# tjiangHIT/cuteSV

Measured on NVIDIA H100. Metric: sv_signatures_clustered_per_sec, higher is better.
Workload: dtype int32

## Files before the change

cutesv_b200/csrc/cutesv_b200.cu:

```cuda
#include <cuda_runtime.h>
#include <dlfcn.h>
#include <nccl.h>
#include <stdarg.h>
#include <stdio.h>
#include <stdlib.h>
#include <string.h>

#include <algorithm>
#include <atomic>
#include <string>
#include <vector>

#include "../../include/cutesv_b200.h"
#include "core.h"
#include "devprims.cuh"
#include "host_tables.h"
#include "kernels.cuh"
#include "radix.cuh"
#include "extract.cuh"
#include "scan_core.h"
#include "sa_core.h"

using namespace csv;

// ... 1050 lines not shown
    if (gs != s) {
        CU(cudaEventRecord(c->ev_side_join[side_k], gs));
        CU(cudaStreamWaitEvent(s, c->ev_side_join[side_k], 0));
    }
    stage_end(c, s, CSV_ST_CLUSTER);
    if (L.mark >= 0) { CU(cudaEventRecord(c->kivs[L.mark].b, s)); L.mark = -1; }
    return CSV_OK;
}

static int run_indel(csv_ctx* c, Lane& L, int t, uint32_t kslot_base) {
    SigTable& s = c->sig[t];
    const cudaStream_t st = L.stream;
    const int64_t n = s.n;
    const uint64_t total = c->contig_off[c->n_contigs];
    const int bits = bits_for(total);
    const bool k64 = bits > 32;
    ContigTab ct{c->d_off.as<uint64_t>(), c->d_len_eff.as<int64_t>(), c->n_contigs};
    Counters* ctr = c->counters.as<Counters>();
    TypeJob J;
    memset(&J, 0, sizeof(J));
    J.svtype = t; J.n_host = n; J.n_dev = nullptr;
    J.cp = cluster_params(c->P, t);
    const uint32_t radius = (uint32_t)std::min<int64_t>((int64_t)(J.cp.min_support - 1) * J.cp.bias, 1 << 24);
    const double lambda = (double)n * (2.0 * radius + 2.0 * (1 << BKT_SHIFT)) / (double)std::max<uint64_t>(total, 1);
    const int rb = (int)((radius + (1u << BKT_SHIFT) - 1) >> BKT_SHIFT);
    const bool prefilter = !k64 && c->prefilter_enabled && J.cp.min_support >= 3 && lambda < 0.8 * J.cp.min_support &&
                           n >= (1 << 16) && rb <= BKT_PAD;
    J.iv.rec = nullptr; J.iv.recc = nullptr;
    uint32_t* sidx = nullptr;
    int rc;
    if (prefilter) {
        int W = PART_W_MAX;
        while (W > PART_W_MIN && (int64_t)(total >> W) + 1 < 2 * (int64_t)c->n_sm) W--;
        const int P = (int)(total >> W) + 1;
        const int n_chunks = (int)((n + PART_ROUND - 1) / PART_ROUND);
        const uint32_t ptw = (uint32_t)((n + PART_PAGE - 1) / PART_PAGE) + 1;
        const size_t edge_words = (size_t)PART_MAX * 2 * BKT_PAD, tab_words = PART_MAX + (size_t)P * ptw;
        stage_begin(c, st, CSV_ST_KEYS);
        CU(L.boff.ensure((edge_words + tab_words) * 4, true));
        uint32_t* edge = L.boff.as<uint32_t>();
        uint32_t* fill = edge + edge_words;
        uint32_t* pt = fill + PART_MAX;
        CU(L.keys_a.ensure(((size_t)ptw - 1 + P) * PART_PAGE * 8));
        uint2* pool = (uint2*)L.keys_a.p;
        CU(L.rec_a.ensure((size_t)n * sizeof(IndelRec)));
        CU(cudaMemsetAsync(edge, 0, (size_t)P * 2 * BKT_PAD * 4, st));
        const int is_ins = t == CSV_INS ? 1 : 0;
        if ((((uintptr_t)s.chrom.p) | ((uintptr_t)s.a.p)) & 15)
            return set_err(CSV_E_STATE, "signature columns are not 16 B aligned");
        uint32_t* pool_next = nullptr;
        TileSync ts;
        if ((rc = take_ticket(c->lb, &pool_next)) || (rc = make_sync(c->lb, L.lb_status, st, (size_t)P, &ts))) return rc;
        const size_t smem = pf_smem_bytes(W);
        const int g = std::min(P, resident_grid(c, k_part_filter, 256, smem));
        LAUNCH(c, st, k_part_scatter, n_chunks, PS_THREADS, ps_smem_bytes(), s.chrom.as<int32_t>(), s.a.as<int32_t>(), n, is_ins, ct, W, P,
               rb, pool, fill, pt, ptw, pool_next, edge, &ctr->status);
        stage_end(c, st, CSV_ST_KEYS);
        stage_begin(c, st, CSV_ST_SORT);
        uint32_t* n_pass = &ctr->n_dom[t];
        LAUNCH_PDL(c, st, k_part_filter, g, 256, smem, (const uint2*)pool, fill, pt, ptw, P, W, rb, (uint32_t)J.cp.min_support,
                   (const uint32_t*)edge, L.keys_b.as<uint32_t>(), L.vals_b.as<uint32_t>(), (uint2*)L.rec_a.p, n_pass, ts);
        stage_end(c, st, CSV_ST_SORT);
        if (c->lane_marks) {
            kprof_begin(c, st, t == CSV_DEL ? "back end<DEL>" : "back end<INS>");
            L.mark = (int)c->kivs.size() - 1;
        }
        J.n_dev = n_pass;
        J.keys32 = L.keys_b.as<uint32_t>();
        sidx = L.vals_b.as<uint32_t>();
    } else {
        stage_begin(c, st, CSV_ST_KEYS);
        if (!k64)
            LAUNCH(c, st, (k_indel_keys<uint32_t>), grid_for(c, n, 256), 256, 0, s.chrom.as<int32_t>(), s.a.as<int32_t>(), s.b.as<int32_t>(),
                   s.rid.as<int32_t>(), n, t == CSV_INS ? 1 : 0, ct, L.keys_a.as<uint32_t>(), &ctr->status);
        else
            LAUNCH(c, st, (k_indel_keys<uint64_t>), grid_for(c, n, 256), 256, 0, s.chrom.as<int32_t>(), s.a.as<int32_t>(), s.b.as<int32_t>(),
                   s.rid.as<int32_t>(), n, t == CSV_INS ? 1 : 0, ct, L.keys_a.as<uint64_t>(), &ctr->status);
        stage_end(c, st, CSV_ST_KEYS);
        stage_begin(c, st, CSV_ST_SORT);
        if (!k64) {
            uint32_t* ko = nullptr;
            rc = lane_sort<uint32_t>(c, L, true, n, bits, &ko, &sidx);
            J.keys32 = ko;
        } else {
            uint64_t* ko = nullptr;
            rc = lane_sort<uint64_t>(c, L, true, n, bits, &ko, &sidx);
            J.keys64 = ko;
        }
        if (rc) return rc;
        stage_end(c, st, CSV_ST_SORT);
    }
    J.iv.chrom = s.chrom.as<int32_t>(); J.iv.a = s.a.as<int32_t>(); J.iv.b = s.b.as<int32_t>(); J.iv.rid = s.rid.as<int32_t>();
    J.iv.c = s.has_c ? s.c.as<int32_t>() : nullptr;
    J.iv.sidx = sidx;
    if (!k64 && c->records_enabled && (J.cp.min_support + 31) / 32 + 1 <= HEAD_MAX_NEED_WORDS) {
        const bool with_c = t == CSV_INS && s.has_c;
        CU(L.rec_a.ensure((size_t)n * sizeof(IndelRec)));
        if (with_c) CU(L.recc_a.ensure((size_t)n * 4));
        J.iv.rec = L.rec_a.as<IndelRec>();
        J.iv.recc = with_c ? L.recc_a.as<int32_t>() : nullptr;
    }
    J.iv.is_ins = t == CSV_INS ? 1 : 0;
    J.small_path = c->small_path_enabled ? 1 : 0;
    L.prev_is_chain_kernel = prefilter;
    rc = run_segment_and_cluster(c, L, J, t, kslot_base);
    L.prev_is_chain_kernel = false;
    return rc;
}

static int run_other(csv_ctx* c, Lane& L, int t, uint32_t kslot_base) {
    SigTable& s = c->sig[t];
    const cudaStream_t st = L.stream;
    const int64_t n = s.n;
// ... 537 lines not shown
```

cutesv_b200/csrc/devprims.cuh:

```cuda
#pragma once
#include <cuda_runtime.h>
#include <stdint.h>

namespace csv {

__device__ __forceinline__ void pdl_wait() { asm volatile("griddepcontrol.wait;" ::: "memory"); }
__device__ __forceinline__ void pdl_launch_dependents() { asm volatile("griddepcontrol.launch_dependents;" ::: "memory"); }

__device__ __forceinline__ uint32_t smem_u32(const void* p) { return (uint32_t)__cvta_generic_to_shared(p); }
__device__ __forceinline__ void mbar_init(uint64_t* bar, uint32_t count) {
    asm volatile("mbarrier.init.shared::cta.b64 [%0], %1;" ::"r"(smem_u32(bar)), "r"(count) : "memory");
}
__device__ __forceinline__ void mbar_arrive(uint64_t* bar) {
    asm volatile("mbarrier.arrive.shared::cta.b64 _, [%0];" ::"r"(smem_u32(bar)) : "memory");
}
__device__ __forceinline__ void mbar_expect_tx(uint64_t* bar, uint32_t bytes) {
    asm volatile("mbarrier.arrive.expect_tx.shared::cta.b64 _, [%0], %1;" ::"r"(smem_u32(bar)), "r"(bytes) : "memory");
}
__device__ __forceinline__ void bulk_copy(void* dst, const void* src, uint32_t bytes, uint64_t* bar) {
    asm volatile("cp.async.bulk.shared::cluster.global.mbarrier::complete_tx::bytes [%0], [%1], %2, [%3];" ::"r"(smem_u32(dst)), "l"(src), "r"(bytes),
                 "r"(smem_u32(bar))
                 : "memory");
}
__device__ __forceinline__ void bulk_load(void* dst, const void* src, uint32_t bytes, uint64_t* bar) {
// ... 14 lines not shown


static constexpr uint32_t LB_GEN_LIMIT = 1u << 31;
__device__ __forceinline__ uint64_t lb_word(uint32_t gen, bool inclusive, uint32_t value) {
    return ((uint64_t)gen << 33) | ((uint64_t)inclusive << 32) | value;
}
__device__ __forceinline__ bool lb_ready(uint64_t v, uint32_t gen) { return (uint32_t)(v >> 33) == gen; }
__device__ __forceinline__ bool lb_inclusive(uint64_t v) { return (v >> 32) & 1u; }
__device__ __forceinline__ uint32_t lb_value(uint64_t v) { return (uint32_t)v; }
__device__ __forceinline__ uint64_t lb_load(const uint64_t* p) {
    uint64_t v;
    asm volatile("ld.relaxed.gpu.global.u64 %0, [%1];" : "=l"(v) : "l"(p) : "memory");
    return v;
}
__device__ __forceinline__ void lb_store(uint64_t* p, uint64_t v) {
    asm volatile("st.relaxed.gpu.global.u64 [%0], %1;" ::"l"(p), "l"(v) : "memory");
}

__device__ __forceinline__ void lookback_publish(uint64_t* status, uint32_t gen, int tile, uint32_t local) {
    lb_store(status + tile, lb_word(gen, tile == 0, local));
}

__device__ __forceinline__ uint32_t lookback_wait_warp(uint64_t* status, uint32_t gen, int tile, uint32_t local) {
    const int lane = threadIdx.x & 31;
    if (tile == 0) return 0;
    uint32_t excl = 0;
    int p = tile - 1;
    while (true) {
        const int q = p - lane;
        const uint64_t v = q >= 0 ? lb_load(status + q) : lb_word(gen, true, 0u);
        const bool ready = lb_ready(v, gen);
        const uint32_t nr = __ballot_sync(0xffffffffu, !ready);
        const uint32_t inc = __ballot_sync(0xffffffffu, ready && lb_inclusive(v));
        const int first_nr = nr ? __ffs(nr) - 1 : 32;
        const int first_inc = inc ? __ffs(inc) - 1 : 32;
        const bool done = first_inc < first_nr;
        const int upto = done ? first_inc + 1 : first_nr;
        uint32_t contrib = lane < upto ? lb_value(v) : 0u;
#pragma unroll
        for (int o = 16; o > 0; o >>= 1) contrib += __shfl_xor_sync(0xffffffffu, contrib, o);
        excl += contrib;
        if (done) break;
        p -= upto;
    }
    if (lane == 0) lb_store(status + tile, lb_word(gen, true, excl + local));
    return excl;
}

__device__ __forceinline__ uint32_t lookback_exclusive_warp(uint64_t* status, uint32_t gen, int tile, uint32_t local) {
    if ((threadIdx.x & 31) == 0) lookback_publish(status, gen, tile, local);
    return lookback_wait_warp(status, gen, tile, local);
}

__device__ __forceinline__ uint32_t block_excl_scan_256(uint32_t v, uint32_t* s_warp, uint32_t* total) {
    const int lane = threadIdx.x & 31, warp = threadIdx.x >> 5;
    uint32_t incl = v;
#pragma unroll
    for (int d = 1; d < 32; d <<= 1) {
        uint32_t y = __shfl_up_sync(0xffffffffu, incl, d);
        if (lane >= d) incl += y;
    }
    if (lane == 31) s_warp[warp] = incl;
    __syncthreads();
    if (warp == 0) {
        uint32_t w = lane < 8 ? s_warp[lane] : 0;
        uint32_t wi = w;
#pragma unroll
        for (int d = 1; d < 8; d <<= 1) {
            uint32_t y = __shfl_up_sync(0xffffffffu, wi, d);
            if (lane >= d) wi += y;
        }
        if (lane < 8) s_warp[lane] = wi - w;
        if (lane == 7) s_warp[8] = wi;
    }
    __syncthreads();
    uint32_t r = s_warp[warp] + incl - v;
    *total = s_warp[8];
    __syncthreads();
    return r;
}

__device__ __forceinline__ uint32_t block_reserve_256(uint32_t cnt, uint32_t* counter, uint32_t* s_warp , int parity) {
    const int lane = threadIdx.x & 31, warp = threadIdx.x >> 5;
    uint32_t incl = cnt;
#pragma unroll
    for (int d = 1; d < 32; d <<= 1) {
        const uint32_t y = __shfl_up_sync(0xffffffffu, incl, d);
        if (lane >= d) incl += y;
    }
    uint32_t* part = s_warp + 8 * parity;
    if (lane == 31) part[warp] = incl;
    __syncthreads();
    uint32_t before = 0, total = 0;
#pragma unroll
    for (int i = 0; i < 8; i++) {
        const uint32_t t = part[i];
        before += i < warp ? t : 0u;
        total += t;
    }
    if (threadIdx.x == 0) s_warp[16] = total ? atomicAdd(counter, total) : 0u;
    __syncthreads();
    return s_warp[16] + before + incl - cnt;
}

static constexpr int SEL_THREADS = 256;
static constexpr int SEL_ITEMS = 8;
static constexpr int SEL_TILE = SEL_THREADS * SEL_ITEMS;

struct TileSync {
    uint32_t* ticket;
    uint64_t* status;
    const uint32_t* epoch;
    uint32_t ordinal;
};
static constexpr uint32_t LB_ORDINALS = 1024;
static constexpr uint32_t LB_EPOCH_LIMIT = 1u << 21;
static_assert((uint64_t)LB_EPOCH_LIMIT * LB_ORDINALS <= LB_GEN_LIMIT, "look-back generations must fit 31 bits");
__global__ void __launch_bounds__(256) k_begin(uint32_t* epoch, uint32_t* tickets, int n_tickets, uint32_t* counters, int n_counters,
                                               unsigned long long* cursor) {
    if (threadIdx.x == 0) { *epoch += 1u; *cursor = 0ull; }
    for (int i = threadIdx.x; i < n_tickets; i += 256) tickets[i] = 0u;
    for (int i = threadIdx.x; i < n_counters; i += 256) counters[i] = 0u;
}
__device__ __forceinline__ uint32_t ts_gen(const TileSync& ts) { return (*ts.epoch) * LB_ORDINALS + ts.ordinal; }

template <class Pred>
__global__ void __launch_bounds__(SEL_THREADS) k_select(Pred pred, int64_t n_host, const uint32_t* n_dev, uint32_t* out,
                                                        uint32_t out_cap, uint32_t* out_count, TileSync ts,
                                                        uint32_t* status_word, uint32_t overflow_bit) {
    __shared__ uint32_t s_warp[9];
    __shared__ uint32_t s_tile, s_excl;
    const int64_t n = n_dev ? (int64_t)*n_dev : n_host;
    const uint32_t gen = ts_gen(ts);
    while (true) {
        if (threadIdx.x == 0) s_tile = atomicAdd(ts.ticket, 1u);
        __syncthreads();
        const uint32_t tile = s_tile;
        const int64_t base = (int64_t)tile * SEL_TILE;
        if (base >= n) break;
        const int64_t i0 = base + (int64_t)threadIdx.x * SEL_ITEMS;
        uint32_t flags = 0, cnt = 0;
#pragma unroll
        for (int j = 0; j < SEL_ITEMS; j++) {
            const int64_t i = i0 + j;
            if (i < n && pred(i)) { flags |= 1u << j; cnt++; }
        }
        uint32_t total;
        const uint32_t local = block_excl_scan_256(cnt, s_warp, &total);
        if (threadIdx.x < 32) {
            const uint32_t ex = lookback_exclusive_warp(ts.status, gen, (int)tile, total);
            if (threadIdx.x == 0) {
                s_excl = ex;
                if (base + SEL_TILE >= n) *out_count = ex + total;
            }
        }
        __syncthreads();
        uint32_t o = s_excl + local;
#pragma unroll
        for (int j = 0; j < SEL_ITEMS; j++) {
            if (flags >> j & 1u) {
                if (o < out_cap) out[o] = (uint32_t)(i0 + j);
                else atomicOr(status_word, overflow_bit);
                o++;
            }
        }
        __syncthreads();
    }
}

template <int ITEMS>
__global__ void __launch_bounds__(SEL_THREADS) k_scan_excl(uint32_t* arr, int64_t n_host, const uint32_t* n_dev, const uint32_t* carry_in,
                                                           uint32_t* total_out, TileSync ts) {
    pdl_launch_dependents(); pdl_wait();
    constexpr int TILE = SEL_THREADS * ITEMS;
    __shared__ uint32_t s_warp[9];
    __shared__ uint32_t s_tile, s_excl;
    int64_t n = n_dev ? (int64_t)*n_dev : n_host;
    if (n > n_host) n = n_host;
    const uint32_t carry = carry_in ? *carry_in : 0u;
    const uint32_t gen = ts_gen(ts);
    if (n <= 0) {
        if (total_out && blockIdx.x == 0 && threadIdx.x == 0) *total_out = carry;
        return;
    }
    while (true) {
        if (threadIdx.x == 0) s_tile = atomicAdd(ts.ticket, 1u);
        __syncthreads();
        const uint32_t tile = s_tile;
        const int64_t base = (int64_t)tile * TILE;
        if (base >= n) break;
        const int64_t i0 = base + (int64_t)threadIdx.x * ITEMS;
        uint32_t v[ITEMS], cnt = 0;
        const bool vec = ITEMS == 4 && (((uintptr_t)arr) & 15) == 0 && i0 + ITEMS <= n;
        if (vec) {
            const uint4 x = *reinterpret_cast<const uint4*>(arr + i0);
            v[0] = x.x; v[1] = x.y; v[2] = x.z; v[3] = x.w;
            cnt = x.x + x.y + x.z + x.w;
        } else {
#pragma unroll
            for (int j = 0; j < ITEMS; j++) {
                v[j] = (i0 + j < n) ? arr[i0 + j] : 0u;
                cnt += v[j];
            }
        }
        uint32_t total;
        const uint32_t local = block_excl_scan_256(cnt, s_warp, &total);
        if (threadIdx.x < 32) {
            const uint32_t ex = lookback_exclusive_warp(ts.status, gen, (int)tile, total);
            if (threadIdx.x == 0) {
                s_excl = ex;
                if (total_out && base + TILE >= n) *total_out = carry + ex + total;
            }
        }
        __syncthreads();
        uint32_t run = carry + s_excl + local;
        if (vec) *reinterpret_cast<uint4*>(arr + i0) = make_uint4(run, run + v[0], run + v[0] + v[1], run + v[0] + v[1] + v[2]);
        else {
#pragma unroll
            for (int j = 0; j < ITEMS; j++) {
                if (i0 + j < n) arr[i0 + j] = run;
                run += v[j];
            }
        }
        __syncthreads();
    }
}

}
```

cutesv_b200/csrc/kernels.cuh:

```cuda
#pragma once
#include "core.h"
#include "devprims.cuh"
#include "radix.cuh"
#include <type_traits>

namespace csv {

static constexpr int WARP_M = 128;
static constexpr int BLOCK_M = 2048;
static constexpr int CL_THREADS = 256;

struct TypeJob {
    int svtype;
    int64_t n_host;
    const uint32_t* n_dev;
    const uint32_t* keys32;
    const uint64_t* keys64;
    IndelView iv;
    SortedView sv;
    ClusterParams cp;
    uint32_t kslot_base;
    const uint32_t* kept_start;
    uint32_t* big_list;
    uint32_t* giant_list;
// ... 58 lines not shown
    constexpr int WORDS = SEL_TILE / 32;
    __shared__ uint32_t s_link[HEAD_MAX_NEED_WORDS + WORDS + HEAD_MAX_NEED_WORDS];
    __shared__ uint32_t s_warp[9];
    __shared__ uint32_t s_tile, s_excl, s_aoff;
    __shared__ uint8_t s_msize[SEL_TILE];
    const int64_t n = job_n(J);
    const uint32_t gen = ts_gen(ts);
    const int need = J.cp.min_support;
    const int back = MR.rec ? (need + 31) / 32 + 1 : 0;
    const int fwd = (MR.rec ? max((need + 31) / 32, (REST_SPLIT + 32) / 32) : (need + 31) / 32) + 1;
    const int lane = threadIdx.x & 31, warp = threadIdx.x >> 5;
    while (true) {
        if (threadIdx.x == 0) s_tile = atomicAdd(ts.ticket, 1u);
        __syncthreads();
        const uint32_t tile = s_tile;
        const int64_t base = (int64_t)tile * SEL_TILE;
        if (base >= n) break;
        for (int w0 = warp; w0 < back + WORDS + fwd; w0 += 8 * (SEL_THREADS / 32)) {
            bool l[8];
#pragma unroll
            for (int u = 0; u < 8; u++) {
                const int w = w0 + u * (SEL_THREADS / 32);
                const int64_t i = base + (int64_t)(w - back) * 32 + lane;
                l[u] = (w < back + WORDS + fwd && i > 0 && i < n) ? job_linked(J, i) : false;
            }
#pragma unroll
            for (int u = 0; u < 8; u++) {
                const int w = w0 + u * (SEL_THREADS / 32);
                const uint32_t m = __ballot_sync(0xffffffffu, l[u]);
                if (lane == 0 && w < back + WORDS + fwd) s_link[w] = m;
            }
        }
        if (MR.del_off && warp == SEL_THREADS / 32 - 1) {
            const uint64_t k0 = J.keys32[base], k1 = J.keys32[min(base + SEL_TILE, n) - 1];
            int lo = 0, span = MR.n_contigs;
            while (span > 1) {
                const int step = (span + 31) / 32;
                const bool le = lane * step < span && MR.del_off[lo + lane * step] <= k0;
                const int j = 31 - __clz(__ballot_sync(0xffffffffu, le));
                lo += j * step;
                span = min(step, span - j * step);
            }
            if (lane == 0) s_aoff = k1 < MR.del_off[lo + 1] ? (uint32_t)MR.del_off[lo] : ~0u;
        }
        __syncthreads();
        const int p0 = threadIdx.x * SEL_ITEMS, q0 = back * 32;
        uint32_t flags = 0, cnt = 0;
#pragma unroll
        for (int j = 0; j < SEL_ITEMS; j++) {
            const int p = p0 + j;
            if (base + p < n && chain_head(s_link, q0 + p, need)) { flags |= 1u << j; cnt++; }
        }
        uint32_t total;
        const uint32_t local = block_excl_scan_256(cnt, s_warp, &total);
        if (MR.small_list) {
            uint32_t o = local;
#pragma unroll
            for (int j = 0; j < SEL_ITEMS; j++)
                if (flags >> j & 1u) s_msize[o++] = (uint8_t)chain_size_class(s_link, q0 + p0 + j, REST_SPLIT);
        }
        if (threadIdx.x < 32) {
            const uint32_t ex = lookback_exclusive_warp(ts.status, gen, (int)tile, total);
            if (threadIdx.x == 0) {
                s_excl = ex;
                if (base + SEL_TILE >= n) *out_count = ex + total;
            }
        }
        if (MR.rec) {
            uint32_t mem = 0;
#pragma unroll 1
            for (int j = 0; j < SEL_ITEMS; j++) {
                const int p = threadIdx.x + j * SEL_THREADS;
                if (base + p < n && chain_member(s_link, q0 + p, need)) mem |= 1u << j;
            }
            const uint32_t* __restrict__ sidx = MR.sidx;
            const int32_t *__restrict__ ca = MR.a, *__restrict__ cb = MR.b, *__restrict__ cr = MR.rid, *__restrict__ cc = MR.c;
            IndelRec* __restrict__ rec = MR.rec;
            int32_t* __restrict__ recc = MR.recc;
            const uint32_t aoff = MR.del_off ? s_aoff : ~0u;
            uint32_t bad = 0;
#pragma unroll 1
            for (int j0 = 0; j0 < SEL_ITEMS; j0 += GATHER_GROUP) {
                uint32_t x[GATHER_GROUP];
#pragma unroll
                for (int u = 0; u < GATHER_GROUP; u++)
                    if (mem >> (j0 + u) & 1u) x[u] = sidx[base + threadIdx.x + (j0 + u) * SEL_THREADS];
#pragma unroll
                for (int u = 0; u < GATHER_GROUP; u++) {
                    if (mem >> (j0 + u) & 1u) {
                        const int64_t i = base + threadIdx.x + (j0 + u) * SEL_THREADS;
                        IndelRec r;
                        r.a = aoff != ~0u ? (int32_t)(J.keys32[i] - aoff) : ca[x[u]];
                        r.b = cb[x[u]]; r.rid = cr[x[u]]; r.idx = x[u];
                        const int32_t c5 = cc ? cc[x[u]] : 0;
                        if (r.rid < 0 || r.b < 0 || c5 < 0) bad |= ST_NEG_FIELD;
                        *reinterpret_cast<int4*>(&rec[i]) = *reinterpret_cast<const int4*>(&r);
                        if (recc) recc[i] = c5;
                    }
                }
            }
            if (bad) atomicOr(status_word, bad);
        }
        __syncthreads();
        uint32_t o = s_excl + local;
#pragma unroll
        for (int j = 0; j < SEL_ITEMS; j++) {
            if (flags >> j & 1u) {
// ... 217 lines not shown
            s_warp[lane] = wi - w;
        }
        __syncthreads();
        const uint32_t o = s_warp[warp] + incl - v;
        s_fill[t] = o;
        s_d[t] = r - o;
    }
    const uint32_t k0 = r / PART_PAGE, k1 = v ? (r + v - 1) / PART_PAGE : k0;
    const bool lead = v && r % PART_PAGE != 0;
    const uint32_t np = v ? k1 - k0 + 1 : 0u, own = np - (lead ? 1u : 0u);
    uint32_t* row = pt + (size_t)t * ptw;
    const uint32_t id = own ? atomicAdd(pool_next, own) : 0u;
    uint32_t g = 1;
    if (lead) asm volatile("ld.relaxed.gpu.global.u32 %0, [%1];" : "=r"(g) : "l"(row + k0) : "memory");
    uint32_t base = np;
#pragma unroll
    for (int d = 1; d < 32; d <<= 1) {
        const uint32_t y = __shfl_up_sync(0xffffffffu, base, d);
        if (lane >= d) base += y;
    }
    uint32_t wbase = 0;
    if (lane == 31) wbase = atomicAdd(&s_npg, base);
    base = __shfl_sync(0xffffffffu, wbase, 31) + base - np;
    s_pb[t] = base - k0;
    __syncthreads();
#pragma unroll
    for (int k = 0; k < 4 * PART_ROUND_V; k++) {
        const int q = 4 * ((k >> 2) * PS_THREADS + t) + (k & 3);
        if (q < m) s_st[atomicAdd(&s_fill[key[k] >> W], 1u)] = make_uint2(key[k], (uint32_t)(s0 + q));
    }
    for (uint32_t i = 0; i < own; i++) {
        const uint32_t k = k1 + 1 - own + i;
        asm volatile("st.relaxed.gpu.global.u32 [%0], %1;" ::"l"(row + k), "r"(id + i + 1u) : "memory");
        s_pg[base + k - k0] = id + i;
    }
    if (lead) {
        while (g == 0) {
            __nanosleep(64);
            asm volatile("ld.relaxed.gpu.global.u32 %0, [%1];" : "=r"(g) : "l"(row + k0) : "memory");
        }
        s_pg[base] = g - 1u;
    }
    __syncthreads();
#pragma unroll
    for (int j = 0; j < PART_ROUND / PS_THREADS; j++) {
        const int q = j * PS_THREADS + t;
        if (q >= m) break;
        const uint2 pr = s_st[q];
        const uint32_t p = pr.x >> W, e = (uint32_t)q + s_d[p];
        pool[(size_t)s_pg[s_pb[p] + e / PART_PAGE] * PART_PAGE + e % PART_PAGE] = pr;
    }
}

__global__ void __launch_bounds__(256) k_part_filter(const uint2* __restrict__ pool, uint32_t* __restrict__ fill, uint32_t* __restrict__ pt,
                                                     uint32_t ptw, int P, int W, int rb, uint32_t need, const uint32_t* __restrict__ edge, uint32_t* __restrict__ keys_out,
                                                     uint32_t* __restrict__ idx_out, uint2* __restrict__ spill, uint32_t* n_out, TileSync ts) {
    pdl_launch_dependents(); pdl_wait();
    extern __shared__ __align__(16) uint32_t s_dyn[];
    const int BP = 1 << (W - BKT_SHIFT), LPER = W - BKT_SHIFT - 8, PER = 1 << LPER;
    uint32_t* s_h = s_dyn;
    uint32_t* s_f = s_dyn + BP;
    uint2* s_st = reinterpret_cast<uint2*>(s_dyn + BP + BP / 32);
    __shared__ uint32_t s_warp[9];
    __shared__ uint32_t s_hl[BKT_PAD], s_hr[BKT_PAD];
    __shared__ uint32_t s_big[PF_BIG_CAP], s_cnt[256];
    __shared__ uint32_t s_tile, s_excl, s_nbig;
    const int lane = threadIdx.x & 31, warp = threadIdx.x >> 5;
    const uint32_t gen = ts_gen(ts);
    const uint32_t bmask = BP - 1;
    static_assert(PART_W_MIN - BKT_SHIFT >= 8 && PART_W_MAX - BKT_SHIFT <= 14, "one strip of 1..64 buckets per thread");
    auto phys = [&](uint32_t b) -> uint32_t { return ((b & (PER - 1)) << 8) | (b >> LPER); };
    auto count = [&](int b) -> uint32_t { return s_h[phys(b)]; };
    const int b0 = (int)threadIdx.x * PER;
    while (true) {
        if (threadIdx.x == 0) { s_tile = atomicAdd(ts.ticket, 1u); s_nbig = 0; }
        for (int i = threadIdx.x; i < BP; i += 256) s_h[i] = 0;
        __syncthreads();
        const int p = (int)s_tile;
        if (p >= P) break;
        if (threadIdx.x < 2 * BKT_PAD) {
            const int j = threadIdx.x % BKT_PAD, right = threadIdx.x / BKT_PAD;
            const int q = right ? p + 1 : p - 1;
            const bool ok = q >= 0 && q < P && j < rb;
            (right ? s_hr : s_hl)[j] = ok ? edge[(int64_t)q * 2 * BKT_PAD + (right ? 0 : BKT_PAD) + j] : 0u;
        }
        const uint32_t np = __ldcg(fill + p);
        uint32_t* row = pt + (size_t)p * ptw;
        auto walk = [&](auto f) {
            constexpr int U = 8;
            static_assert(2 * 256 * U == 2 * PART_PAGE, "k_part_filter: two pages per step");
            for (uint32_t k = 0; 2 * PART_PAGE * k < np; k++) {
                const uint32_t e0 = 2 * PART_PAGE * k + 2 * threadIdx.x;
                const uint2* pg0 = pool + (size_t)(__ldg(row + 2 * k) - 1u) * PART_PAGE;
                const uint2* pg1 = PART_PAGE * (2 * k + 1) < np ? pool + (size_t)(__ldg(row + 2 * k + 1) - 1u) * PART_PAGE : pg0;
                uint4 v[U];
#pragma unroll
                for (int u = 0; u < U; u++) {
                    const uint32_t e = e0 + 2 * 256 * u;
                    v[u] = e < np ? __ldg(reinterpret_cast<const uint4*>((2 * 256 * u + 2 * threadIdx.x < PART_PAGE ? pg0 : pg1) + e % PART_PAGE))
                                  : make_uint4(0u, 0u, 0u, 0u);
                }
#pragma unroll
                for (int u = 0; u < U; u++) {
                    const uint32_t e = e0 + 2 * 256 * u;
                    if (e < np) f(make_uint2(v[u].x, v[u].y));
                    if (e + 1 < np) f(make_uint2(v[u].z, v[u].w));
                }
            }
        };
        walk([&](uint2 pr) { atomicAdd(&s_h[phys((pr.x >> BKT_SHIFT) & bmask)], 1u); });
        __syncthreads();
        uint32_t kept, S;
        const uint64_t flags = pf_strip_flags(count, [&](int s, int j) -> uint32_t { return s_h[(j << 8) + (int)threadIdx.x + s]; },
                                              b0, PER, BP, rb, need, s_hl, s_hr, &kept);
        const uint32_t first = block_excl_scan_256(kept, s_warp, &S);
        if (threadIdx.x == 0) {
            lookback_publish(ts.status, gen, p, S);
            if (S) atomicAdd(n_out, S);
        }
        const bool spilled = S > (uint32_t)PF_STAGE;
        if (spilled && warp == 0) {
            const uint32_t ex = lookback_wait_warp(ts.status, gen, p, S);
            if (lane == 0) s_excl = ex;
        }
        pf_strip_offsets([&](int b) -> uint32_t { return s_h[((b - b0) << 8) | threadIdx.x]; }, b0, PER, flags, first,
                         [&](int j, uint32_t off, bool f, uint32_t c) {
            s_h[(j << 8) | threadIdx.x] = off;
            const uint32_t bits = __ballot_sync(0xffffffffu, f);
            if (lane == 0) s_f[(j << 3) | warp] = bits;
            if (c > FIX_SMALL) {
                const uint32_t q = atomicAdd(&s_nbig, 1u);
                if (q < PF_BIG_CAP) s_big[q] = (uint32_t)(b0 + j);
            }
        });
        __syncthreads();
        if (!spilled && warp == 0) {
            const uint32_t ex = lookback_wait_warp(ts.status, gen, p, S);
            if (lane == 0) s_excl = ex;
        }
        uint2* st = spilled ? spill + s_excl : s_st;
        walk([&](uint2 pr) {
            const uint32_t ph = phys((pr.x >> BKT_SHIFT) & bmask);
            if ((s_f[ph >> 5] >> (ph & 31)) & 1u) st[atomicAdd(&s_h[ph], 1u)] = pr;
        });
        __syncthreads();
        for (uint32_t k = threadIdx.x; k < (np + PART_PAGE - 1) / PART_PAGE; k += 256) row[k] = 0u;
        if (threadIdx.x == 0) fill[p] = 0u;
        const uint32_t obase = s_excl;
        for (uint32_t q = threadIdx.x; q < S; q += 256) {
            const uint2 pr = st[q];
            const uint32_t b = (pr.x >> BKT_SHIFT) & bmask;
            const uint32_t beg = b ? s_h[phys(b - 1)] : 0u, end = s_h[phys(b)];
            if (end - beg > FIX_SMALL) continue;
            uint32_t rank = 0;
            for (uint32_t j = beg; j < end; j++) {
                const uint32_t k = st[j].x;
                rank += (k < pr.x || (k == pr.x && j < q)) ? 1u : 0u;
            }
            keys_out[obase + beg + rank] = pr.x;
            idx_out[obase + beg + rank] = pr.y;
        }
        static_assert((1 << BKT_SHIFT) == 256, "one counting-sort bin per thread");
        const uint32_t nbig = s_nbig;
        const uint32_t nb = nbig <= (uint32_t)PF_BIG_CAP ? nbig : (uint32_t)BP;
        for (uint32_t k = 0; k < nb; k++) {
            const uint32_t b = nbig <= (uint32_t)PF_BIG_CAP ? s_big[k] : k;
            const uint32_t beg = b ? s_h[phys(b - 1)] : 0u, end = s_h[phys(b)];
            if (end - beg <= FIX_SMALL) continue;
            __syncthreads();
            s_cnt[threadIdx.x] = 0;
            __syncthreads();
            for (uint32_t j = beg + threadIdx.x; j < end; j += 256) atomicAdd(&s_cnt[st[j].x & 255u], 1u);
            __syncthreads();
            uint32_t total;
            const uint32_t ex = block_excl_scan_256(s_cnt[threadIdx.x], s_warp, &total);
            s_cnt[threadIdx.x] = ex;
            __syncthreads();
            for (uint32_t j = beg + threadIdx.x; j < end; j += 256) {
                const uint2 pr = st[j];
                const uint32_t d = obase + beg + atomicAdd(&s_cnt[pr.x & 255u], 1u);
                keys_out[d] = pr.x;
                idx_out[d] = pr.y;
            }
        }
        __syncthreads();
    }
}

template <bool TRA_PAIR>
__global__ void k_other_keys(const int32_t* __restrict__ chrom, const int32_t* __restrict__ a, const int32_t* __restrict__ b,
                             const int32_t* __restrict__ rid, const int32_t* __restrict__ c, int64_t n, int svtype, ContigTab ct,
                             uint32_t* __restrict__ k_rid, uint32_t* __restrict__ k_b, uint64_t* __restrict__ k_prim,
                             uint32_t* status) {
    for (int64_t i = (int64_t)blockIdx.x * blockDim.x + threadIdx.x; i < n; i += (int64_t)gridDim.x * blockDim.x) {
        uint32_t bad = 0;
        const int32_t ch = chrom[i], ai = a[i], bi = b[i], ri = rid[i], ci = c ? c[i] : 0;
        if (ch < 0 || ch >= ct.n) bad |= ST_BAD_CHROM;
        else if (ct.len[ch] < 0) bad |= ST_BAD_POS;
        if (ai < 0 || bi < 0 || ri < 0 || ci < 0) bad |= ST_NEG_FIELD;
        if (svtype == CSV_TRA && (ci >> 2) >= ct.n) bad |= ST_BAD_CHROM;
        if (svtype == CSV_INV && ci > 1) bad |= ST_NEG_FIELD;
        if (bad) atomicOr(status, bad);
        if (k_rid) { k_rid[i] = (uint32_t)ri; k_b[i] = (uint32_t)bi; }
        uint64_t hi = (uint64_t)(uint32_t)ch;
        if (svtype == CSV_INV) hi = hi * 2 + (uint32_t)ci;
        if (svtype == CSV_TRA) hi = hi * (uint64_t)(4 * ct.n) + (uint32_t)ci;
        k_prim[i] = TRA_PAIR ? hi : (hi << 31) | (uint32_t)ai;
    }
}

__global__ void k_tra_pair_flags(const uint64_t* __restrict__ pair_sorted, int64_t n, uint32_t* __restrict__ flag) {
    for (int64_t i = (int64_t)blockIdx.x * blockDim.x + threadIdx.x; i < n; i += (int64_t)gridDim.x * blockDim.x)
        flag[i] = (i + 1 < n && pair_sorted[i + 1] != pair_sorted[i]) ? 1u : 0u;
}
__global__ void k_tra_compact_key(const uint32_t* __restrict__ perm, const uint32_t* __restrict__ rank, const int32_t* __restrict__ a,
                                  int64_t n, uint64_t* __restrict__ k_prim) {
    for (int64_t i = (int64_t)blockIdx.x * blockDim.x + threadIdx.x; i < n; i += (int64_t)gridDim.x * blockDim.x) {
        const uint32_t x = perm[i];
        k_prim[x] = ((uint64_t)rank[i] << 31) | (uint32_t)a[x];
    }
}

static constexpr int RUN_MAX = 2048;
__global__ void __launch_bounds__(256) k_run_fixup(const uint64_t* __restrict__ kprim_sorted, const uint32_t* __restrict__ perm, int64_t n,
                                                   const int32_t* __restrict__ b, const int32_t* __restrict__ rid,
                                                   uint32_t* __restrict__ perm_out, uint32_t* status) {
    for (int64_t i = (int64_t)blockIdx.x * blockDim.x + threadIdx.x; i < n; i += (int64_t)gridDim.x * blockDim.x) {
        const uint64_t k = kprim_sorted[i];
        const uint32_t x = perm[i];
        const bool alone = (i == 0 || kprim_sorted[i - 1] != k) && (i + 1 >= n || kprim_sorted[i + 1] != k);
        if (alone) { perm_out[i] = x; continue; }
// ... 866 lines not shown
```

cutesv_b200/csrc/radix.cuh:

```cuda
#pragma once
#include "devprims.cuh"

namespace csv {

static constexpr int RS_THREADS = 256;
static constexpr int RS_WARPS = RS_THREADS / 32;
static constexpr int RS_MAX_PASSES = 8;

__device__ __forceinline__ uint32_t match_digit8(uint32_t d) {
    uint32_t ret = 0xffffffffu;
#pragma unroll
    for (int b = 0; b < 8; b++) {
        uint32_t mask;
        asm volatile(
            "{\n"
            "  .reg .pred p;\n"
            "  and.b32 %0, %1, %2;\n"
            "  setp.ne.u32 p, %0, 0;\n"
            "  vote.sync.ballot.b32 %0, p, 0xffffffff;\n"
            "  @!p not.b32 %0, %0;\n"
            "}\n"
            : "=r"(mask)
            : "r"(d), "r"(1u << b));
        ret &= mask;
    }
    return ret;
}

template <typename K> struct RsTraits;
template <> struct RsTraits<uint32_t> { static constexpr int ITEMS = 16; };
template <> struct RsTraits<uint64_t> { static constexpr int ITEMS = 12; };

template <typename K>
__global__ void __launch_bounds__(RS_THREADS) k_rs_hist(const K* __restrict__ keys, int64_t n_host, const uint32_t* n_dev,
                                                        int passes, uint32_t* __restrict__ hist) {
    __shared__ uint32_t s_hist[RS_MAX_PASSES * 256];
    const int64_t n = n_dev ? (int64_t)*n_dev : n_host;
    for (int i = threadIdx.x; i < passes * 256; i += RS_THREADS) s_hist[i] = 0;
    __syncthreads();
    for (int64_t i = (int64_t)blockIdx.x * RS_THREADS + threadIdx.x; i < n; i += (int64_t)gridDim.x * RS_THREADS) {
        const K k = keys[i];
        for (int p = 0; p < passes; p++) atomicAdd(&s_hist[p * 256 + (int)((k >> (8 * p)) & 0xff)], 1u);
    }
    __syncthreads();
    for (int i = threadIdx.x; i < passes * 256; i += RS_THREADS) {
        const uint32_t v = s_hist[i];
        if (v) atomicAdd(&hist[i], v);
    }
}

__global__ void __launch_bounds__(256) k_rs_hist_scan(uint32_t* hist, int passes) {
    __shared__ uint32_t s_warp[9];
    for (int p = 0; p < passes; p++) {
        const uint32_t v = hist[p * 256 + threadIdx.x];
        uint32_t total;
        const uint32_t e = block_excl_scan_256(v, s_warp, &total);
        hist[p * 256 + threadIdx.x] = e;
    }
}

template <typename K, bool IOTA>
__global__ void __launch_bounds__(RS_THREADS, 4) k_rs_onesweep(const K* __restrict__ keys_in, const uint32_t* __restrict__ vals_in,
                                                            K* __restrict__ keys_out, uint32_t* __restrict__ vals_out,
                                                            int64_t n_host, const uint32_t* n_dev, int shift,
                                                            const uint32_t* __restrict__ gbase, TileSync ts) {
    constexpr int ITEMS = RsTraits<K>::ITEMS;
    constexpr int TILE = RS_THREADS * ITEMS;
    __shared__ uint32_t s_warp_hist[RS_WARPS][256];
    __shared__ uint32_t s_excl[256];
    __shared__ int64_t s_dst[256];
    __shared__ K s_keys[TILE];
    __shared__ uint32_t s_vals[TILE];
    __shared__ uint32_t s_scan[9];
    __shared__ uint32_t s_tile;

    const int64_t n = n_dev ? (int64_t)*n_dev : n_host;
    const uint32_t gen = ts_gen(ts);
    uint64_t* const status = ts.status;
    const int tid = threadIdx.x, lane = tid & 31, warp = tid >> 5;
    if (tid == 0) s_tile = atomicAdd(ts.ticket, 1u);
    for (int i = tid; i < RS_WARPS * 256; i += RS_THREADS) (&s_warp_hist[0][0])[i] = 0;
    __syncthreads();
    const int tile = (int)s_tile;
    const int64_t base = (int64_t)tile * TILE;
    if (base >= n) return;
    const int n_valid = (int)((n - base) < TILE ? (n - base) : TILE);

    K k[ITEMS];
    uint32_t rank[ITEMS];
    const int wbase = warp * 32 * ITEMS;
#pragma unroll
    for (int i = 0; i < ITEMS; i++) {
        const int p = wbase + i * 32 + lane;
        k[i] = p < n_valid ? keys_in[base + p] : (K)~(K)0;
    }
    uint32_t pm[ITEMS];
#pragma unroll
    for (int i = 0; i < ITEMS; i++) pm[i] = match_digit8((uint32_t)((k[i] >> shift) & 0xff));
#pragma unroll
    for (int i = 0; i < ITEMS; i++) {
        const int d = (int)((k[i] >> shift) & 0xff);
        const uint32_t peers = pm[i];
        const int leader = __ffs(peers) - 1;
        uint32_t prev = 0;
        if (lane == leader) {
            prev = s_warp_hist[warp][d];
            s_warp_hist[warp][d] = prev + __popc(peers);
        }
        prev = __shfl_sync(0xffffffffu, prev, leader);
        rank[i] = prev + __popc(peers & ((1u << lane) - 1u));
        __syncwarp();
    }
    __syncthreads();
    {
        const int d = tid;
        uint32_t sum = 0;
#pragma unroll
        for (int w = 0; w < RS_WARPS; w++) {
            const uint32_t t = s_warp_hist[w][d];
            s_warp_hist[w][d] = sum;
            sum += t;
        }
        uint32_t total;
        const uint32_t excl_local = block_excl_scan_256(sum, s_scan, &total);
        s_excl[d] = excl_local;
        uint64_t* st = status + d;
        uint32_t excl_tiles = 0;
        if (tile == 0) {
            lb_store(st, lb_word(gen, true, sum));
        } else {
            lb_store(st + (size_t)tile * 256, lb_word(gen, false, sum));
            constexpr int LB_BATCH = 8;
            int p = tile - 1;
            bool done = false;
            while (!done) {
                uint64_t v[LB_BATCH];
#pragma unroll
                for (int j = 0; j < LB_BATCH; j++) {
                    const int q = p - j;
                    v[j] = q >= 0 ? lb_load(st + (size_t)q * 256) : lb_word(gen, true, 0u);
                }
                int used = 0;
#pragma unroll
                for (int j = 0; j < LB_BATCH; j++) {
                    if (!done && used == j && lb_ready(v[j], gen)) {
                        excl_tiles += lb_value(v[j]);
                        used = j + 1;
                        if (lb_inclusive(v[j])) done = true;
                    }
                }
                p -= used;
            }
            lb_store(st + (size_t)tile * 256, lb_word(gen, true, excl_tiles + sum));
        }
        s_dst[d] = (int64_t)gbase[d] + (int64_t)excl_tiles - (int64_t)excl_local;
    }
    __syncthreads();
#pragma unroll
    for (int i = 0; i < ITEMS; i++) {
        const int p = wbase + i * 32 + lane;
        const int d = (int)((k[i] >> shift) & 0xff);
        const uint32_t pos = s_excl[d] + s_warp_hist[warp][d] + rank[i];
        s_keys[pos] = k[i];
        uint32_t v = 0;
        if (p < n_valid) v = IOTA ? (uint32_t)(base + p) : vals_in[base + p];
        s_vals[pos] = v;
    }
    __syncthreads();
#pragma unroll
    for (int i = 0; i < ITEMS; i++) {
        const int p = i * RS_THREADS + tid;
        if (p < n_valid) {
            const K key = s_keys[p];
            const int d = (int)((key >> shift) & 0xff);
            const int64_t dst = s_dst[d] + p;
            keys_out[dst] = key;
            vals_out[dst] = s_vals[p];
// ... 6 lines not shown
```

Baseline: 19.91 billion.

## Widen k_part_filter to 512-thread CTAs with four-page walk steps

Generalizes the block exclusive scan to a templated CTA width and raises k_part_filter from 256 to 512 threads per block, with launch bounds asking for two resident blocks per SM. Bucket strip mapping, the keep-flag layout and the page walk (now four pages per step) are reworked for the wider block, and threads beyond the bucket count own no strip. The aim is more parallelism and memory-level concurrency per partition tile. The cost is extra register pressure from the launch bounds and idle threads when the bucket count is small.

Result: faster. 21.14 billion, median of 6 (+6.2%).

```diff
diff --git a/cutesv_b200/csrc/cutesv_b200.cu b/cutesv_b200/csrc/cutesv_b200.cu
--- a/cutesv_b200/csrc/cutesv_b200.cu
+++ b/cutesv_b200/csrc/cutesv_b200.cu
@@ -1126,13 +1126,13 @@
         TileSync ts;
         if ((rc = take_ticket(c->lb, &pool_next)) || (rc = make_sync(c->lb, L.lb_status, st, (size_t)P, &ts))) return rc;
         const size_t smem = pf_smem_bytes(W);
-        const int g = std::min(P, resident_grid(c, k_part_filter, 256, smem));
+        const int g = std::min(P, resident_grid(c, k_part_filter, PF_THREADS, smem));
         LAUNCH(c, st, k_part_scatter, n_chunks, PS_THREADS, ps_smem_bytes(), s.chrom.as<int32_t>(), s.a.as<int32_t>(), n, is_ins, ct, W, P,
                rb, pool, fill, pt, ptw, pool_next, edge, &ctr->status);
         stage_end(c, st, CSV_ST_KEYS);
         stage_begin(c, st, CSV_ST_SORT);
         uint32_t* n_pass = &ctr->n_dom[t];
-        LAUNCH_PDL(c, st, k_part_filter, g, 256, smem, (const uint2*)pool, fill, pt, ptw, P, W, rb, (uint32_t)J.cp.min_support,
+        LAUNCH_PDL(c, st, k_part_filter, g, PF_THREADS, smem, (const uint2*)pool, fill, pt, ptw, P, W, rb, (uint32_t)J.cp.min_support,
                    (const uint32_t*)edge, L.keys_b.as<uint32_t>(), L.vals_b.as<uint32_t>(), (uint2*)L.rec_a.p, n_pass, ts);
         stage_end(c, st, CSV_ST_SORT);
         if (c->lane_marks) {
diff --git a/cutesv_b200/csrc/devprims.cuh b/cutesv_b200/csrc/devprims.cuh
--- a/cutesv_b200/csrc/devprims.cuh
+++ b/cutesv_b200/csrc/devprims.cuh
@@ -90,7 +90,10 @@
     return lookback_wait_warp(status, gen, tile, local);
 }
 
-__device__ __forceinline__ uint32_t block_excl_scan_256(uint32_t v, uint32_t* s_warp, uint32_t* total) {
+template <int NT>
+__device__ __forceinline__ uint32_t block_excl_scan(uint32_t v, uint32_t* s_warp, uint32_t* total) {
+    static_assert(NT % 32 == 0 && NT >= 64 && NT <= 1024, "block_excl_scan: whole warps, at most 32");
+    constexpr int NW = NT / 32;
     const int lane = threadIdx.x & 31, warp = threadIdx.x >> 5;
     uint32_t incl = v;
 #pragma unroll
@@ -101,19 +104,19 @@
     if (lane == 31) s_warp[warp] = incl;
     __syncthreads();
     if (warp == 0) {
-        uint32_t w = lane < 8 ? s_warp[lane] : 0;
+        uint32_t w = lane < NW ? s_warp[lane] : 0;
         uint32_t wi = w;
 #pragma unroll
-        for (int d = 1; d < 8; d <<= 1) {
+        for (int d = 1; d < NW; d <<= 1) {
             uint32_t y = __shfl_up_sync(0xffffffffu, wi, d);
             if (lane >= d) wi += y;
         }
-        if (lane < 8) s_warp[lane] = wi - w;
-        if (lane == 7) s_warp[8] = wi;
+        if (lane < NW) s_warp[lane] = wi - w;
+        if (lane == NW - 1) s_warp[NW] = wi;
     }
     __syncthreads();
     uint32_t r = s_warp[warp] + incl - v;
-    *total = s_warp[8];
+    *total = s_warp[NW];
     __syncthreads();
     return r;
 }
@@ -184,7 +187,7 @@
             if (i < n && pred(i)) { flags |= 1u << j; cnt++; }
         }
         uint32_t total;
-        const uint32_t local = block_excl_scan_256(cnt, s_warp, &total);
+        const uint32_t local = block_excl_scan<256>(cnt, s_warp, &total);
         if (threadIdx.x < 32) {
             const uint32_t ex = lookback_exclusive_warp(ts.status, gen, (int)tile, total);
             if (threadIdx.x == 0) {
@@ -242,7 +245,7 @@
             }
         }
         uint32_t total;
-        const uint32_t local = block_excl_scan_256(cnt, s_warp, &total);
+        const uint32_t local = block_excl_scan<256>(cnt, s_warp, &total);
         if (threadIdx.x < 32) {
             const uint32_t ex = lookback_exclusive_warp(ts.status, gen, (int)tile, total);
             if (threadIdx.x == 0) {
diff --git a/cutesv_b200/csrc/kernels.cuh b/cutesv_b200/csrc/kernels.cuh
--- a/cutesv_b200/csrc/kernels.cuh
+++ b/cutesv_b200/csrc/kernels.cuh
@@ -134,7 +134,7 @@
             if (base + p < n && chain_head(s_link, q0 + p, need)) { flags |= 1u << j; cnt++; }
         }
         uint32_t total;
-        const uint32_t local = block_excl_scan_256(cnt, s_warp, &total);
+        const uint32_t local = block_excl_scan<256>(cnt, s_warp, &total);
         if (MR.small_list) {
             uint32_t o = local;
 #pragma unroll
@@ -458,29 +458,35 @@
     }
 }
 
-__global__ void __launch_bounds__(256) k_part_filter(const uint2* __restrict__ pool, uint32_t* __restrict__ fill, uint32_t* __restrict__ pt,
+static constexpr int PF_THREADS = 512, PF_LT = 9;
+static_assert(PF_THREADS == 1 << PF_LT, "k_part_filter: a power-of-two CTA");
+static_assert((1 << (PART_W_MAX - BKT_SHIFT)) / PF_THREADS <= 64, "k_part_filter: a strip's keep flags fit one 64-bit word");
+static_assert((1 << (PART_W_MIN - BKT_SHIFT)) % 32 == 0,
+              "k_part_filter: below PF_THREADS buckets, one bucket per thread; whole warps own a strip or none");
+__global__ void __launch_bounds__(PF_THREADS, 2) k_part_filter(const uint2* __restrict__ pool, uint32_t* __restrict__ fill, uint32_t* __restrict__ pt,
                                                      uint32_t ptw, int P, int W, int rb, uint32_t need, const uint32_t* __restrict__ edge, uint32_t* __restrict__ keys_out,
                                                      uint32_t* __restrict__ idx_out, uint2* __restrict__ spill, uint32_t* n_out, TileSync ts) {
     pdl_launch_dependents(); pdl_wait();
     extern __shared__ __align__(16) uint32_t s_dyn[];
-    const int BP = 1 << (W - BKT_SHIFT), LPER = W - BKT_SHIFT - 8, PER = 1 << LPER;
+    const int BP = 1 << (W - BKT_SHIFT);
+    const int LPER = W - BKT_SHIFT > PF_LT ? W - BKT_SHIFT - PF_LT : 0, PER = 1 << LPER;
     uint32_t* s_h = s_dyn;
     uint32_t* s_f = s_dyn + BP;
     uint2* s_st = reinterpret_cast<uint2*>(s_dyn + BP + BP / 32);
-    __shared__ uint32_t s_warp[9];
+    __shared__ uint32_t s_warp[PF_THREADS / 32 + 1];
     __shared__ uint32_t s_hl[BKT_PAD], s_hr[BKT_PAD];
     __shared__ uint32_t s_big[PF_BIG_CAP], s_cnt[256];
     __shared__ uint32_t s_tile, s_excl, s_nbig;
     const int lane = threadIdx.x & 31, warp = threadIdx.x >> 5;
     const uint32_t gen = ts_gen(ts);
     const uint32_t bmask = BP - 1;
-    static_assert(PART_W_MIN - BKT_SHIFT >= 8 && PART_W_MAX - BKT_SHIFT <= 14, "one strip of 1..64 buckets per thread");
-    auto phys = [&](uint32_t b) -> uint32_t { return ((b & (PER - 1)) << 8) | (b >> LPER); };
+    auto phys = [&](uint32_t b) -> uint32_t { return ((b & (PER - 1)) << PF_LT) | (b >> LPER); };
     auto count = [&](int b) -> uint32_t { return s_h[phys(b)]; };
     const int b0 = (int)threadIdx.x * PER;
+    const int nst = (int)threadIdx.x < BP ? PER : 0;
     while (true) {
         if (threadIdx.x == 0) { s_tile = atomicAdd(ts.ticket, 1u); s_nbig = 0; }
-        for (int i = threadIdx.x; i < BP; i += 256) s_h[i] = 0;
+        for (int i = threadIdx.x; i < BP; i += PF_THREADS) s_h[i] = 0;
         __syncthreads();
         const int p = (int)s_tile;
         if (p >= P) break;
@@ -494,21 +500,22 @@
         uint32_t* row = pt + (size_t)p * ptw;
         auto walk = [&](auto f) {
             constexpr int U = 8;
-            static_assert(2 * 256 * U == 2 * PART_PAGE, "k_part_filter: two pages per step");
-            for (uint32_t k = 0; 2 * PART_PAGE * k < np; k++) {
-                const uint32_t e0 = 2 * PART_PAGE * k + 2 * threadIdx.x;
-                const uint2* pg0 = pool + (size_t)(__ldg(row + 2 * k) - 1u) * PART_PAGE;
-                const uint2* pg1 = PART_PAGE * (2 * k + 1) < np ? pool + (size_t)(__ldg(row + 2 * k + 1) - 1u) * PART_PAGE : pg0;
+            static_assert(2 * PF_THREADS * U == 4 * PART_PAGE && 2 * PF_THREADS * 2 == PART_PAGE, "k_part_filter: four pages per step, two loads per page");
+            for (uint32_t k = 0; 4 * PART_PAGE * k < np; k++) {
+                const uint32_t e0 = 4 * PART_PAGE * k + 2 * threadIdx.x;
+                uint32_t pg[4];
+#pragma unroll
+                for (int i = 0; i < 4; i++) pg[i] = PART_PAGE * (4 * k + i) < np ? __ldg(row + 4 * k + i) - 1u : 0u;
                 uint4 v[U];
 #pragma unroll
                 for (int u = 0; u < U; u++) {
-                    const uint32_t e = e0 + 2 * 256 * u;
-                    v[u] = e < np ? __ldg(reinterpret_cast<const uint4*>((2 * 256 * u + 2 * threadIdx.x < PART_PAGE ? pg0 : pg1) + e % PART_PAGE))
+                    const uint32_t e = e0 + 2 * PF_THREADS * u;
+                    v[u] = e < np ? __ldg(reinterpret_cast<const uint4*>(pool + (size_t)pg[u >> 1] * PART_PAGE + e % PART_PAGE))
                                   : make_uint4(0u, 0u, 0u, 0u);
                 }
 #pragma unroll
                 for (int u = 0; u < U; u++) {
-                    const uint32_t e = e0 + 2 * 256 * u;
+                    const uint32_t e = e0 + 2 * PF_THREADS * u;
                     if (e < np) f(make_uint2(v[u].x, v[u].y));
                     if (e + 1 < np) f(make_uint2(v[u].z, v[u].w));
                 }
@@ -516,10 +523,11 @@
         };
         walk([&](uint2 pr) { atomicAdd(&s_h[phys((pr.x >> BKT_SHIFT) & bmask)], 1u); });
         __syncthreads();
-        uint32_t kept, S;
-        const uint64_t flags = pf_strip_flags(count, [&](int s, int j) -> uint32_t { return s_h[(j << 8) + (int)threadIdx.x + s]; },
-                                              b0, PER, BP, rb, need, s_hl, s_hr, &kept);
-        const uint32_t first = block_excl_scan_256(kept, s_warp, &S);
+        uint32_t kept = 0, S;
+        const uint64_t flags = nst ? pf_strip_flags(count, [&](int s, int j) -> uint32_t { return s_h[(j << PF_LT) + (int)threadIdx.x + s]; },
+                                                    b0, PER, BP, rb, need, s_hl, s_hr, &kept)
+                                   : 0ull;
+        const uint32_t first = block_excl_scan<PF_THREADS>(kept, s_warp, &S);
         if (threadIdx.x == 0) {
             lookback_publish(ts.status, gen, p, S);
             if (S) atomicAdd(n_out, S);
@@ -529,11 +537,11 @@
             const uint32_t ex = lookback_wait_warp(ts.status, gen, p, S);
             if (lane == 0) s_excl = ex;
         }
-        pf_strip_offsets([&](int b) -> uint32_t { return s_h[((b - b0) << 8) | threadIdx.x]; }, b0, PER, flags, first,
+        pf_strip_offsets([&](int b) -> uint32_t { return s_h[((b - b0) << PF_LT) | threadIdx.x]; }, b0, nst, flags, first,
                          [&](int j, uint32_t off, bool f, uint32_t c) {
-            s_h[(j << 8) | threadIdx.x] = off;
+            s_h[(j << PF_LT) | threadIdx.x] = off;
             const uint32_t bits = __ballot_sync(0xffffffffu, f);
-            if (lane == 0) s_f[(j << 3) | warp] = bits;
+            if (lane == 0) s_f[(j << (PF_LT - 5)) | warp] = bits;
             if (c > FIX_SMALL) {
                 const uint32_t q = atomicAdd(&s_nbig, 1u);
                 if (q < PF_BIG_CAP) s_big[q] = (uint32_t)(b0 + j);
@@ -550,10 +558,10 @@
             if ((s_f[ph >> 5] >> (ph & 31)) & 1u) st[atomicAdd(&s_h[ph], 1u)] = pr;
         });
         __syncthreads();
-        for (uint32_t k = threadIdx.x; k < (np + PART_PAGE - 1) / PART_PAGE; k += 256) row[k] = 0u;
+        for (uint32_t k = threadIdx.x; k < (np + PART_PAGE - 1) / PART_PAGE; k += PF_THREADS) row[k] = 0u;
         if (threadIdx.x == 0) fill[p] = 0u;
         const uint32_t obase = s_excl;
-        for (uint32_t q = threadIdx.x; q < S; q += 256) {
+        for (uint32_t q = threadIdx.x; q < S; q += PF_THREADS) {
             const uint2 pr = st[q];
             const uint32_t b = (pr.x >> BKT_SHIFT) & bmask;
             const uint32_t beg = b ? s_h[phys(b - 1)] : 0u, end = s_h[phys(b)];
@@ -566,7 +574,7 @@
             keys_out[obase + beg + rank] = pr.x;
             idx_out[obase + beg + rank] = pr.y;
         }
-        static_assert((1 << BKT_SHIFT) == 256, "one counting-sort bin per thread");
+        static_assert((1 << BKT_SHIFT) == 256 && PF_THREADS >= 256, "one counting-sort bin per thread of the first 256");
         const uint32_t nbig = s_nbig;
         const uint32_t nb = nbig <= (uint32_t)PF_BIG_CAP ? nbig : (uint32_t)BP;
         for (uint32_t k = 0; k < nb; k++) {
@@ -574,15 +582,15 @@
             const uint32_t beg = b ? s_h[phys(b - 1)] : 0u, end = s_h[phys(b)];
             if (end - beg <= FIX_SMALL) continue;
             __syncthreads();
-            s_cnt[threadIdx.x] = 0;
+            if (threadIdx.x < 256) s_cnt[threadIdx.x] = 0;
             __syncthreads();
-            for (uint32_t j = beg + threadIdx.x; j < end; j += 256) atomicAdd(&s_cnt[st[j].x & 255u], 1u);
+            for (uint32_t j = beg + threadIdx.x; j < end; j += PF_THREADS) atomicAdd(&s_cnt[st[j].x & 255u], 1u);
             __syncthreads();
             uint32_t total;
-            const uint32_t ex = block_excl_scan_256(s_cnt[threadIdx.x], s_warp, &total);
-            s_cnt[threadIdx.x] = ex;
+            const uint32_t ex = block_excl_scan<PF_THREADS>(threadIdx.x < 256 ? s_cnt[threadIdx.x] : 0u, s_warp, &total);
+            if (threadIdx.x < 256) s_cnt[threadIdx.x] = ex;
             __syncthreads();
-            for (uint32_t j = beg + threadIdx.x; j < end; j += 256) {
+            for (uint32_t j = beg + threadIdx.x; j < end; j += PF_THREADS) {
                 const uint2 pr = st[j];
                 const uint32_t d = obase + beg + atomicAdd(&s_cnt[pr.x & 255u], 1u);
                 keys_out[d] = pr.x;
diff --git a/cutesv_b200/csrc/radix.cuh b/cutesv_b200/csrc/radix.cuh
--- a/cutesv_b200/csrc/radix.cuh
+++ b/cutesv_b200/csrc/radix.cuh
@@ -54,7 +54,7 @@
     for (int p = 0; p < passes; p++) {
         const uint32_t v = hist[p * 256 + threadIdx.x];
         uint32_t total;
-        const uint32_t e = block_excl_scan_256(v, s_warp, &total);
+        const uint32_t e = block_excl_scan<256>(v, s_warp, &total);
         hist[p * 256 + threadIdx.x] = e;
     }
 }
@@ -122,7 +122,7 @@
             sum += t;
         }
         uint32_t total;
-        const uint32_t excl_local = block_excl_scan_256(sum, s_scan, &total);
+        const uint32_t excl_local = block_excl_scan<256>(sum, s_scan, &total);
         s_excl[d] = excl_local;
         uint64_t* st = status + d;
         uint32_t excl_tiles = 0;
```
